# Angtian/VoGE

Hardware: AMD Instinct MI355X
Metric: forward+backward frames/sec at 512^2, 50k Gaussians; ray-trace HBM GB/s vs peak (higher is better)
Workload: dtype f32; 1 GPU; cfg3_50k_512: 50000 random Gaussians (scalar sigmas), 512x512, K=40, max_point_per_bin=-1, fwd+bwd (grads to verts, sigmas, colors); launch=hip graph replay, 4 consecutive steps per graph launch, parallelism=1 gpu

## Files before the change

### __graft_entry__.py

```python
import os
import subprocess
import sys

ROOT = os.path.dirname(os.path.abspath(__file__))
if ROOT not in sys.path:
    sys.path.insert(0, ROOT)


def build() -> None:
    subprocess.check_call(["make", "-C", os.path.join(ROOT, "voge_amd", "csrc"), "-B", "-j2", "all"])
    import oracle
    oracle.build(force=True)
    import voge_amd
    lib = voge_amd.load_library()
    assert lib.voge_abi_version() == 7
    from oracle import build_ref
    build_ref.build(force=True)


def smoke() -> None:
    import numpy as np
    import torch
    import oracle
    from oracle import camera_np
    from voge_amd.Meshes import GaussianMeshes
    from voge_amd.Renderer import GaussianRenderer, GaussianRenderSettings, to_white_background
    from voge_amd.cameras import PerspectiveCameras
    from voge_amd import scenes

    assert torch.cuda.is_available(), "smoke() needs a HIP device"
    dev = "cuda:0"
    verts, sig, cols = scenes.random_gaussians(600, seed=1, r_lo=0.08, r_hi=0.16)
    H = W = 64
    R, T = camera_np.look_at_view_transform(3.5, 15.0, 40.0)
    cams = PerspectiveCameras(focal_length=60.0, principal_point=((32.0, 32.0),), image_size=((H, W),), device=dev)
    st = GaussianRenderSettings(image_size=(H, W), max_assign=16, max_point_per_bin=-1)
    renderer = GaussianRenderer(cams, st).to(dev)
    gm = GaussianMeshes(torch.from_numpy(verts), torch.from_numpy(sig)).to(dev)
    colors = torch.from_numpy(cols).to(dev).requires_grad_(True)
    frag = renderer(gm, R=torch.from_numpy(R).to(dev), T=torch.from_numpy(T).to(dev))
    img = to_white_background(frag, colors)
    img.sum().backward()
    torch.cuda.synchronize()
    ref = oracle.render(verts, sig, cols, R, T, 60.0, (32.0, 32.0), (H, W), K=16)
    same = (frag.vert_index.cpu().numpy() == np.where(ref["idx"] < 0, 0, ref["idx"])).all(-1)
    err = np.abs(img.detach().cpu().numpy() - ref["image"])[same].max()
    assert same.mean() > 0.99 and err < 1e-4, (same.mean(), err)
    assert torch.isfinite(gm.verts.grad).all() and gm.verts.grad.abs().max() > 0
    print(f"smoke ok: {same.mean() * 100:.2f}% pixels identical index lists, max image err {err:.2e}")


if __name__ == "__main__":
    build()
    if len(sys.argv) > 1 and sys.argv[1] == "smoke":
        smoke()
```

### voge_amd/ops.py

```python
import math
import os
import struct

import torch

from . import _lib


_raw_stream = getattr(torch._C, "_cuda_getCurrentRawStream", None)
_get_dev = getattr(torch._C, "_cuda_getDevice", None) or torch.cuda.current_device
_set_dev = getattr(torch._C, "_cuda_setDevice", None) or torch.cuda.set_device


def _stream():
    if _raw_stream is not None:
        return _raw_stream(_get_dev())
    return torch.cuda.current_stream().cuda_stream


class _on:
    __slots__ = ("idx", "prev")

    def __init__(self, device):
        self.idx = device.index if device.index is not None else _get_dev()
        self.prev = -1

    def __enter__(self):
        cur = _get_dev()
        if cur != self.idx:
            self.prev = cur
            _set_dev(self.idx)

    def __exit__(self, *exc):
        if self.prev >= 0:
            _set_dev(self.prev)
        return False


def _dev(t, dtype, name):
    if not isinstance(t, torch.Tensor):
        raise TypeError(f"{name} must be a torch.Tensor")
    if not t.is_cuda:
        raise _lib.VogeHipError(
            f"{name} is on {t.device}: the VoGE hot path runs on a HIP device only (no CPU fallback)")
    if t.dtype != dtype:
        t = t.to(dtype)
    return t.contiguous()


def _p(t):
    return None if t is None else t.data_ptr()


_WS = {}


def _workspace(dev, nbytes):
    nbytes = max(int(nbytes), 16)
    if torch.cuda.is_current_stream_capturing():
        return torch.empty((nbytes,), dtype=torch.uint8, device=dev)
    key = (dev.index if dev.index is not None else _get_dev(), _stream())
    ws = _WS.get(key)
    if ws is None or ws.numel() < nbytes:
        ws = _WS[key] = torch.empty((nbytes,), dtype=torch.uint8, device=dev)
    return ws


def release_workspaces(device=None):
    idx = None if device is None else (torch.device(device).index if torch.device(device).index is not None else _get_dev())
    for key in [k for k in _WS if idx is None or k[0] == idx]:
        del _WS[key]


class _GeneralPreamble(torch.autograd.Function):

    @staticmethod
    def forward(ctx, verts, sigmas, origin):
        lib = _lib.load()
        v_c, s_c, o_c = _dev(verts, torch.float32, "verts"), _dev(sigmas, torch.float32, "sigmas"), _dev(origin, torch.float32, "origin")
        B = o_c.shape[0]
        shared_v = v_c.dim() == 2
        N = v_c.shape[-2]
        kind = 2 if tuple(s_c.shape[-2:]) == (3, 3) and s_c.dim() >= 3 else 1
        shared_s = s_c.dim() == (3 if kind == 2 else 2)
        assert v_c.shape[-1] == 3 and (shared_v or v_c.shape[0] == B) and o_c.shape == (B, 3)
        assert s_c.shape[-1] == 3 and s_c.shape[-(kind + 1)] == N and (shared_s or s_c.shape[0] == B)
        mus = torch.empty((B * N, 3), dtype=torch.float32, device=v_c.device)
        isg = torch.empty((B * N, 3, 3), dtype=torch.float32, device=v_c.device)
        with _on(v_c.device):
            rc = lib.voge_general_preamble_fwd(_p(v_c), _p(s_c), _p(o_c), B, N, int(shared_v), int(shared_s), kind, _p(mus), _p(isg),
                                               _stream())
        _lib.check(rc, "voge_general_preamble_fwd")
        ctx.meta = (B, N, shared_v, shared_s, kind, tuple(v_c.shape), tuple(s_c.shape))
        ctx.set_materialize_grads(False)
        return mus, isg

    @staticmethod
    def backward(ctx, g_mus, g_isg):
        lib = _lib.load()
        B, N, shared_v, shared_s, kind, vshape, sshape = ctx.meta
        if ctx.needs_input_grad[2]:
            raise _lib.VogeHipError("the fused preamble carries no gradient for the camera centre")
        g_v = g_s = None
        gm = None if g_mus is None else _dev(g_mus, torch.float32, "grad_mus")
        ga = None if g_isg is None else _dev(g_isg, torch.float32, "grad_isigmas")
        dev = (gm if gm is not None else ga)
        if dev is None:
            return None, None, None
        dev = dev.device
        if ctx.needs_input_grad[0] and gm is not None:
            g_v = torch.empty(vshape, dtype=torch.float32, device=dev)
        if ctx.needs_input_grad[1] and ga is not None:
            g_s = torch.empty(sshape, dtype=torch.float32, device=dev)
        if g_v is not None or g_s is not None:
            with _on(dev):
                rc = lib.voge_general_preamble_bwd(_p(gm if g_v is not None else None), _p(ga if g_s is not None else None), B, N,
                                                   int(shared_v), int(shared_s), kind, _p(g_v), _p(g_s), _stream())
            _lib.check(rc, "voge_general_preamble_bwd")
        return g_v, g_s, None


def general_preamble(verts, sigmas, origin):
    return _GeneralPreamble.apply(verts, sigmas, origin)


def trace_pool_usage(dev, B, N, H, W):
    import ctypes
    lib = _lib.load()
    dev = torch.device(dev)
    with _on(dev):
        nbytes = lib.voge_trace_workspace_bytes(B, N, H, W)
        ws = _workspace(dev, nbytes)
        used, cap = ctypes.c_int(0), ctypes.c_int(0)
        torch.cuda.current_stream(dev).synchronize()
        _lib.check(lib.voge_trace_pool_usage(_p(ws), nbytes, B, N, H, W, ctypes.byref(used), ctypes.byref(cap)), "voge_trace_pool_usage")
    return used.value, cap.value


def _tag_index(sel_idx, cnt, n_index):
    if cnt is not None:
        sel_idx.voge_hit_count = (cnt, sel_idx._version)
    sel_idx.voge_index_bound = (int(n_index), sel_idx._version)


def carry_tags(src, dst):
    if dst is src or not (isinstance(dst, torch.Tensor) and dst.is_cuda and dst.is_contiguous()
                          and dst.data_ptr() == src.data_ptr() and dst.numel() == src.numel() and dst.dtype == src.dtype):
        return dst
    tag = getattr(src, "voge_hit_count", None)
    if tag is not None:
        dst.voge_hit_count = (tag[0].view(dst.shape[:-1]), tag[1])
    for name in ("voge_index_bound", "voge_through"):
        tag = getattr(src, name, None)
        if tag is not None:
# ... 315 lines not shown
        lib = _lib.load()
        act, dsd = torch.empty_like(ln), torch.empty_like(ln)
        K = idx.shape[-1]
        with _on(ln.device):
            rc = lib.voge_fragment_act_dsd_iso(_p(records), _p(rays), _p(idx), _p(ln), _p(cnt), idx.numel() // K, K, P,
                                               _p(act), _p(dsd), _stream())
        _lib.check(rc, "voge_fragment_act_dsd_iso")
        cell[0], cell[1] = act, dsd
    return cell[0], cell[1]


def fragments(mode, p0, p1, origin, rays, cam_fwd, thr_act, n_assign, sigma_mode=0, occ=1.0):
    weight, sel_idx, valid, sel_len, cnt, records, sel_act, sel_dsd = _Fragments.apply(
        mode, p0, p1, origin, rays, cam_fwd, thr_act, n_assign, sigma_mode, occ)
    if (p0.requires_grad or p1.requires_grad) and torch.is_grad_enabled():
        B = rays.shape[0]
        N = p0.shape[-2] if mode == 2 else p0.shape[0] // max(B, 1)
        rays_d, len_d = rays.detach(), sel_len.detach()
        weight.voge_through = dict(
            mode=int(mode), sigma_mode=int(sigma_mode), shared=bool(mode == 2 and p0.dim() == 2), occ=float(occ), B=B, N=N,
            records=records, rays=rays_d, act=sel_act, dsd=sel_dsd, len=len_d, cnt=cnt, idx=sel_idx,
            sigmas=p1.detach(), means=p0.detach(), p0=p0, p1=p1, rays_requires_grad=bool(rays.requires_grad),
            versions=(weight._version, len_d._version, rays_d._version, sel_idx._version))
    return weight, sel_idx, valid, sel_len


LAZY_COMPOSITE = os.environ.get("VOGE_LAZY_COMPOSITE", "1") != "0"


class _TraceLean(torch.autograd.Function):

    @staticmethod
    def forward(ctx, mode, p0, p1, origin, rays, cam_fwd, thr_act, n_assign, sigma_mode):
        p0_c, p1_c, o_c, rays_c, fwd, B, N, H, W, shared = _trace_inputs(mode, p0, p1, origin, rays, cam_fwd)
        K, dev = int(n_assign), rays_c.device
        sel_idx = torch.empty((B, H, W, K), dtype=torch.int32, device=dev)
        sel_len = torch.empty((B, H, W, K), dtype=torch.float32, device=dev)
        cnt = torch.empty((B, H, W), dtype=torch.int32, device=dev)
        records = torch.empty((B * N, 12 if mode == 0 else 4), dtype=torch.float32, device=dev)
        _sweep(mode, p0_c, p1_c, o_c, shared, sigma_mode, rays_c, fwd, B, N, H, W, K, thr_act, 1.0, sel_idx, sel_len, None, None, cnt,
               None, None, records)
        ctx.save_for_backward(p0_c, p1_c, rays_c, sel_len)
        ctx.sel_idx, ctx.cnt, ctx.records = sel_idx, cnt, records
        ctx.meta = (int(mode), int(sigma_mode), bool(shared), B, N)
        _tag_index(sel_idx, cnt, B * N)
        ctx.mark_non_differentiable(sel_idx, cnt, records)
        ctx.set_materialize_grads(False)
        return sel_idx, sel_len, cnt, records

    @staticmethod
    def backward(ctx, _g_idx, g_len, _g_cnt, _g_rec):
        if g_len is None:
            return (None,) * 9
        p0, p1, rays, ln = ctx.saved_tensors
        mode, sigma_mode, shared, B, N = ctx.meta
        if ctx.needs_input_grad[4] or ctx.needs_input_grad[3]:
            raise _lib.VogeHipError("deferred-composite fragments carry no gradient for the rays / the camera centre; "
                                    "VOGE_LAZY_COMPOSITE=0 (or rays that require grad at render time) selects the eager chain")
        g0, g1 = _fragment_bwd(mode, p0, p1, ctx.records, shared, sigma_mode, rays, ctx.sel_idx, ctx.cnt, B, N, (p0, p1), ln, None, ln,
                               None, None, g_len, 1.0)
        return None, g0, g1, None, None, None, None, None, None


def _plain(t_, dtype, name):
    if not t_.is_cuda:
        raise _lib.VogeHipError(f"{name} is on {t_.device}: the VoGE hot path runs on a HIP device only (no CPU fallback)")
    if t_.dtype != dtype or not t_.is_contiguous():
        t_ = t_.detach().to(dtype).contiguous()
    return t_


def _sigma_kind(sigmas):
    kind = 2 if tuple(sigmas.shape[-2:]) == (3, 3) and sigmas.dim() >= 3 else 1
    return kind, sigmas.dim() == (3 if kind == 2 else 2)


def _plain16(t_, name):
    t_ = _plain(t_, torch.float32, name)
    return t_ if t_.data_ptr() % 16 == 0 else t_.detach().clone()


def _frame_trace(verts, sigmas, R, T, focal, pp, band, W, behind, thr_act, n_assign, sigma_mode, occ, origin_out, gen, quats=None):
    lib = _lib.load()
    v_c, s_c = _plain(verts, torch.float32, "verts"), _plain(sigmas, torch.float32, "sigmas")
    R_c, T_c = _plain(R, torch.float32, "R"), _plain(T, torch.float32, "T")
    f_c, p_c = _plain(focal, torch.float32, "focal_length"), _plain(pp, torch.float32, "principal_point")
    B = R_c.shape[0]
    row0, h, stripe_h, pitch = band
    shared = v_c.dim() == 2
    N, K, dev = v_c.shape[-2], int(n_assign), v_c.device
    assert R_c.shape == (B, 3, 3) and T_c.shape == (B, 3) and f_c.shape == (B, 2) and p_c.shape == (B, 2)
    assert v_c.shape[-1] == 3 and (shared or v_c.shape[0] == B)
    if quats is not None:
        q_c = _plain16(quats, "quats")
        shared_s = s_c.dim() == 2
        assert tuple(s_c.shape[-2:]) == (N, 3) and q_c.shape == s_c.shape[:-1] + (4,) and (shared_s or s_c.shape[0] == B)
        assert sigma_mode in (1, 2)
        nrec, form = 12, (0, int(sigma_mode), False, (3, int(shared), int(shared_s)))
    elif gen:
        kind, shared_s = _sigma_kind(s_c)
        assert s_c.shape[-(kind + 1)] == N and s_c.shape[-1] == 3 and (shared_s or s_c.shape[0] == B)
        nrec, form = (8 if kind == 1 else 12), (0, 0, False, (kind, int(shared), int(shared_s)))
    else:
        assert s_c.shape == v_c.shape[:-1]
        nrec, form = 4, (2, int(sigma_mode), shared, None)
    empty = torch.empty
    sel_idx = empty((B, h, W, K), dtype=torch.int32, device=dev)
    sel_len = empty((B, h, W, K), dtype=torch.float32, device=dev)
    cnt = empty((B, h, W), dtype=torch.int32, device=dev)
    records = empty((B * N, nrec), dtype=torch.float32, device=dev)
    rays = empty((B, h, W, 3), dtype=torch.float32, device=dev)
    with _on(dev):
        nbytes = lib.voge_trace_workspace_bytes(B, N, h, W)
        ws = _workspace(dev, nbytes)
        cam = (R_c.data_ptr(), T_c.data_ptr(), f_c.data_ptr(), p_c.data_ptr(), int(row0), int(stripe_h), int(pitch), int(bool(behind)), B,
               N, int(h), int(W), K, float(thr_act), ws.data_ptr(), nbytes, sel_idx.data_ptr(), sel_len.data_ptr(), cnt.data_ptr(),
               records.data_ptr(), rays.data_ptr(), _p(origin_out), _stream())
        if quats is not None:
            rc = lib.voge_frame_trace_fwd_ori(v_c.data_ptr(), s_c.data_ptr(), q_c.data_ptr(), int(shared), int(shared_s), int(sigma_mode), *cam)
        elif gen:
            rc = lib.voge_frame_trace_fwd_gen(v_c.data_ptr(), s_c.data_ptr(), int(shared), int(shared_s), kind, *cam)
        else:
            rc = lib.voge_frame_trace_fwd_iso(v_c.data_ptr(), s_c.data_ptr(), int(shared), int(sigma_mode), *cam)
    if rc:
        _lib.check(rc, "voge_frame_trace_fwd")
    _tag_index(sel_idx, cnt, B * N)
    lz = LazyComposite.__new__(LazyComposite)
    lz.mode, lz.sigma_mode, lz.shared, lz.gen = form
    (lz.occ, lz.B, lz.N, lz.K, lz.p0, lz.p1, lz.sel_idx, lz.sel_len, lz.cnt, lz.records, lz.rays, lz.rays_version, lz.grad_mode,
     lz.idx_version, lz.p0_version, lz.frame) = (float(occ), B, N, K, verts, sigmas, sel_idx, sel_len, cnt, records, rays, 0,
                                                 torch.is_grad_enabled(), sel_idx._version, verts._version, True)
    lz.p2 = quats
    lz.p12_version = None if quats is None else (sigmas._version, quats._version)
    return sel_idx, sel_len, lz


def frame_trace(verts, sigmas, R, T, focal, pp, band, W, behind, thr_act, n_assign, sigma_mode, occ, origin_out=None):
    return _frame_trace(verts, sigmas, R, T, focal, pp, band, W, behind, thr_act, n_assign, sigma_mode, occ, origin_out, False)


def frame_trace_gen(verts, sigmas, R, T, focal, pp, band, W, behind, thr_act, n_assign, occ, origin_out=None):
    return _frame_trace(verts, sigmas, R, T, focal, pp, band, W, behind, thr_act, n_assign, 0, occ, origin_out, True)


def frame_trace_ori(verts, scales, quats, R, T, focal, pp, band, W, behind, thr_act, n_assign, sigma_mode, occ, origin_out=None):
    return _frame_trace(verts, scales, R, T, focal, pp, band, W, behind, thr_act, n_assign, sigma_mode, occ, origin_out, True, quats)


def _frame_gen_bwd(lz, form, attr, weight, ad, ln, rgb, wsum, bg, thr, g, gs0, gs1, g_hitlen, acc=None):
    lz.check()
    lib = _lib.load()
    kind, shared_v, shared_s = lz.gen
    dev = ln.device
    B, H, W = lz.cnt.shape
    K, P = lz.K, lz.B * lz.N
    g0 = torch.empty(lz.p0.shape, dtype=torch.float32, device=dev)
    g1 = torch.empty(lz.p1.shape, dtype=torch.float32, device=dev)
    g_attr = None if attr is None else torch.empty_like(attr)
    g2 = None
    C, Nattr = (0, 0) if attr is None else (attr.shape[1], attr.shape[0])
    with _on(dev):
        zeroed = acc is not None
        if acc is None:
            nbytes = lib.voge_frame_bwd_gen_acc_bytes(P)
            acc = _workspace(dev, nbytes)
        else:
            nbytes = acc.numel()
        tail = (_p(lz.rays), _p(attr), _p(lz.sel_idx), _p(lz.cnt), _p(weight), _p(ad[0]), _p(ln), _p(ad[1]), _p(rgb), _p(wsum), _p(bg),
                float(thr), _p(g), gs0, gs1, _p(g_hitlen), lz.occ, lz.B, lz.N, B * H, W, K, C, Nattr, _p(acc), nbytes, int(zeroed), _p(g0),
                _p(g1))
        if kind == 3:
            g2 = torch.empty(lz.p2.shape, dtype=torch.float32, device=dev)
            rc = lib.voge_frame_bwd_ori(form, _p(lz.records), _p(_plain(lz.p1, torch.float32, "scales")), _p(_plain16(lz.p2, "quats")),
                                        shared_v, shared_s, lz.sigma_mode, *tail, _p(g2), _p(g_attr), _stream())
        else:
            rc = lib.voge_frame_bwd_gen(form, _p(lz.records), shared_v, shared_s, kind, *tail, _p(g_attr), _stream())
    _lib.check(rc, "voge_frame_bwd_ori" if kind == 3 else "voge_frame_bwd_gen")
    return g0, g1, g2, g_attr


class _HitLength(torch.autograd.Function):

    @staticmethod
    def forward(ctx, p0, p1, sel_len, lz, p2=None):
        ctx.lz = lz
        ctx.save_for_backward(p1)
        ctx.set_materialize_grads(False)
        return sel_len.view_as(sel_len)

    @staticmethod
    def backward(ctx, g_len):
        if g_len is None:
            return None, None, None, None, None
        lz = ctx.lz
        (p1,) = ctx.saved_tensors
        if lz.gen is None:
            p1 = _dev(p1, torch.float32, "sigmas")
        g0, g1, g2 = _lazy_fragment_bwd(lz, p1, lz.sel_len, lz.sel_len, None, g_len=g_len, occ=1.0)
        return g0, g1, None, None, g2


FRAME_PATH = os.environ.get("VOGE_FRAME_PATH", "1") != "0"
FRAME_DIRECT_BWD = os.environ.get("VOGE_FRAME_DIRECT_BWD", "1") != "0"


def frame_eligible(verts, sigmas, R, T, focal, pp, n_assign, numel):
    if not (LAZY_COMPOSITE and FRAME_PATH) or n_assign > _lib.MAX_K or os.environ.get("VOGE_FRAGMENTS_KEEP_ACT_DSD", "0") == "1":
        return False
# ... 106 lines not shown
            per = 32 if lz.gen is None else (48 if lz.gen[0] == 1 else 64)
        return torch.empty((lz.B * lz.N * per,), dtype=torch.uint8, device=lz.sel_idx.device)
    return None


def _composite_fwd(lz, sel_len, need, attr=None, bg=None, thr=-1.0, rgb=None, img=None, wsum=None, sil=None, acc=None):
    lib = _lib.load()
    idx, K = lz.sel_idx, lz.K
    npix = idx.numel() // K
    C, Nattr = (0, 0) if attr is None else (attr.shape[1], attr.shape[0])
    nacc = 0 if acc is None else acc.numel()
    weight = torch.empty_like(sel_len)
    valid = torch.empty(idx.shape[:-1], dtype=torch.int64, device=idx.device)
    with _on(idx.device):
        ad = _general_act_dsd(lz, sel_len, need)
        src = (_p(idx), _p(lz.cnt), _p(sel_len), _p(lz.records), _p(lz.rays), lz.occ)
        args = src + (_p(attr), _p(bg), float(thr), npix, K, C, Nattr, _p(weight), _p(valid), _p(rgb), _p(img), _p(wsum))
        if lz.gen is not None:
            rc = lib.voge_frame_shade_fwd_rec(1 if lz.gen[0] == 1 else 2, *args, _p(sil), _p(ad[0]), _p(ad[1]), _p(acc), nacc, _stream())
        elif attr is None and lz.mode == 0:
            rc = lib.voge_composite_fwd_rec(*src, npix, K, _p(weight), _p(valid), _p(ad[0]), _p(ad[1]), _stream())
        elif attr is None:
            rc = lib.voge_composite_fwd_iso(*src, npix, K, _p(weight), _p(valid), _stream())
        elif lz.mode == 0:
            rc = lib.voge_composite_shade_fwd_rec(*args, _p(ad[0]), _p(ad[1]), _stream())
        elif sil is not None or acc is not None:
            rc = lib.voge_frame_shade_fwd_iso(*args, _p(sil), _p(acc), nacc, _stream())
        else:
            rc = lib.voge_composite_shade_fwd_iso(*args, _stream())
    _lib.check(rc, "voge_composite_fwd (from the records)")
    weight.voge_act_dsd = ad
    return weight, valid, ad


class _CompositeLean(torch.autograd.Function):

    @staticmethod
    def forward(ctx, p0, p1, sel_len, lz, p2=None):
        weight, valid, ctx.ad = _composite_fwd(lz, sel_len, any(ctx.needs_input_grad))
        ctx.save_for_backward(_dev(p1, torch.float32, "sigmas"), sel_len, weight)
        ctx.lz = lz
        ctx.mark_non_differentiable(valid)
        ctx.set_materialize_grads(False)
        return weight, valid

    @staticmethod
    def backward(ctx, g_weight, _g_valid):
        if g_weight is None:
            return None, None, None, None, None
        p1, ln, weight = ctx.saved_tensors
        g0, g1, g2 = _lazy_fragment_bwd(ctx.lz, p1, weight, ln, g_weight, ctx.ad)
        return g0, g1, None, None, g2


def _shade_bwd(mode, means, sigmas, records, shared, sigma_mode, rays, cnt, occ, B, N, like, attr, idx, weight, act, ln, dsd, rgb,
               wsum, bg, thr, go, gs_pix, gs_c, acc=None):
    lib = _lib.load()
    _, H, W, K = idx.shape
    Nattr, C = attr.shape
    dev = idx.device
    g_attr = torch.empty_like(attr)
    g0 = torch.empty(like[0].shape, dtype=torch.float32, device=dev)
    g1 = torch.empty(like[1].shape, dtype=torch.float32, device=dev)
    image = (_p(rgb), _p(wsum), _p(bg), thr, _p(go), gs_pix, gs_c, occ)
    sizes = (B * H, W, K, C, Nattr)
    grads = (_p(g0), _p(g1), _p(g_attr))
    with _on(dev):
        if acc is not None:
            rc = lib.voge_frame_shade_bwd_iso(_p(records), _p(sigmas), int(shared), sigma_mode, _p(rays), _p(attr), _p(idx), _p(cnt),
                                              _p(weight), _p(ln), *image, B, N, *sizes, _p(acc), acc.numel(), *grads, _stream())
        else:
            nbytes = lib.voge_fragment_bwd_workspace_bytes(B * N)
            ws = _workspace(dev, nbytes)
            slots = (_p(attr), _p(idx), _p(cnt), _p(weight), _p(act), _p(ln), _p(dsd), *image)
            if mode == 0:
                rc = lib.voge_fragment_shade_bwd(_p(means), _p(sigmas), _p(rays), *slots, B * N, *sizes, _p(ws), nbytes, *grads, _stream())
            else:
                rc = lib.voge_fragment_shade_bwd_iso(_p(records), _p(sigmas), int(shared), sigma_mode, _p(rays), *slots, B, N, *sizes,
                                                     _p(ws), nbytes, *grads, _stream())
    _lib.check(rc, "voge_fragment_shade_bwd")
    return g0, g1, g_attr


class _CompositeShade(torch.autograd.Function):

    @staticmethod
    def forward(ctx, attr, p0, p1, sel_len, lz, bg, thr, p2=None):
        attr_c = _dev(attr, torch.float32, "colors")
        bg_c = _dev(bg, torch.float32, "background_color")
        idx = lz.sel_idx
        Nattr, C = attr_c.shape
        assert bg_c.numel() == C
        check_index_range(idx, Nattr)
        rgb = torch.empty(idx.shape[:-1] + (C,), dtype=torch.float32, device=idx.device)
        img = torch.empty_like(rgb)
        wsum = torch.empty(idx.shape[:-1], dtype=torch.float32, device=idx.device)
        ctx.gbuf = _frame_acc(lz, any(ctx.needs_input_grad[:3]) or ctx.needs_input_grad[-1])
        weight, valid, ctx.ad = _composite_fwd(lz, sel_len, any(ctx.needs_input_grad), attr_c, bg_c, thr, rgb, img, wsum, acc=ctx.gbuf)
        ctx.save_for_backward(attr_c, _dev(p1, torch.float32, "sigmas"), sel_len, weight, rgb, bg_c, wsum)
        ctx.lz, ctx.thr = lz, float(thr)
        ctx.mark_non_differentiable(valid)
        ctx.set_materialize_grads(False)
        return img, weight, valid

    @staticmethod
    def backward(ctx, g_img, g_weight, _g_valid):
        attr, p1, ln, weight, rgb, bg, wsum = ctx.saved_tensors
        lz = ctx.lz
        lz.check()
        g_attr = g0 = g1 = g2 = None
        if g_img is not None:
            go, gs_pix, gs_c = _grad_layout(g_img, attr.shape[1])
            gbuf, ctx.gbuf = ctx.gbuf, None
            if lz.gen is not None:
                g0, g1, g2, g_attr = _frame_gen_bwd(lz, 0, attr, weight, ctx.ad, ln, rgb, wsum, bg, ctx.thr, go, gs_pix, gs_c, None, acc=gbuf)
            else:
                g0, g1, g_attr = _shade_bwd(lz.mode, lz.means() if lz.mode == 0 else None, p1, lz.records, lz.shared, lz.sigma_mode,
                                            lz.rays, lz.cnt, lz.occ, lz.B, lz.N, (lz.p0, lz.p1), attr, lz.sel_idx, weight, ctx.ad[0], ln,
                                            ctx.ad[1], rgb, wsum, bg, ctx.thr, go, gs_pix, gs_c, gbuf)
        if g_weight is not None:
            h0, h1, h2 = _lazy_fragment_bwd(lz, p1, weight, ln, g_weight, ctx.ad)
            g0, g1, g2 = (h0, h1, h2) if g0 is None else (g0 + h0, g1 + h1, None if h2 is None else g2 + h2)
        need = ctx.needs_input_grad
        return ((g_attr if need[0] else None), (g0 if need[1] else None), (g1 if need[2] else None), None, None, None, None,
                (g2 if need[7] else None))


def _merge_bwd(lz, p1, attr, weight, ad, ln, go, gs_pix, gs_c, gws, wsum_fwd, acc):
    lib = _lib.load()
    idx = lz.sel_idx
    B, H, W, K = idx.shape
    Nattr, C = attr.shape
    dev = idx.device
    g_attr = torch.empty_like(attr)
    g0 = torch.empty(lz.p0.shape, dtype=torch.float32, device=dev)
    g1 = torch.empty(lz.p1.shape, dtype=torch.float32, device=dev)
    grad = (_p(go), gs_pix, gs_c, _p(gws))
    sizes = (B * H, W, K, C, Nattr)
    grads = (_p(g0), _p(g1), _p(g_attr))
    with _on(dev):
        if acc is not None:
            rc = lib.voge_frame_merge_bwd_iso(_p(lz.records), _p(p1), int(lz.shared), lz.sigma_mode, _p(lz.rays), _p(attr), _p(idx),
                                              _p(lz.cnt), _p(weight), _p(ln), *grad, _p(wsum_fwd), lz.occ, lz.B, lz.N, *sizes, _p(acc),
                                              acc.numel(), *grads, _stream())
        else:
            nbytes = lib.voge_fragment_bwd_workspace_bytes(lz.B * lz.N)
            ws = _workspace(dev, nbytes)
            slots = (_p(attr), _p(idx), _p(lz.cnt), _p(weight), _p(ad[0]), _p(ln), _p(ad[1]), *grad, lz.occ)
            if lz.mode == 0:
                rc = lib.voge_fragment_merge_bwd(_p(lz.means()), _p(p1), _p(lz.rays), *slots, lz.B * lz.N, *sizes, _p(ws), nbytes, *grads,
                                                 _stream())
            else:
                rc = lib.voge_fragment_merge_bwd_iso(_p(lz.records), _p(p1), int(lz.shared), lz.sigma_mode, _p(lz.rays), *slots, lz.B,
                                                     lz.N, *sizes, _p(ws), nbytes, *grads, _stream())
    _lib.check(rc, "voge_fragment_merge_bwd")
    return g0, g1, g_attr


class _CompositeMerge(torch.autograd.Function):

    @staticmethod
    def forward(ctx, attr, p0, p1, sel_len, lz, p2=None):
        attr_c = _dev(attr, torch.float32, "vert_attr")
        idx = lz.sel_idx
        Nattr, C = attr_c.shape
        check_index_range(idx, Nattr)
        rgb = torch.empty(idx.shape[:-1] + (C,), dtype=torch.float32, device=idx.device)
        wsum = torch.empty(idx.shape[:-1], dtype=torch.float32, device=idx.device)
        sil = torch.empty_like(wsum) if lz.frame else None
        ctx.gbuf = _frame_acc(lz, any(ctx.needs_input_grad[:3]) or ctx.needs_input_grad[-1])
        weight, valid, ctx.ad = _composite_fwd(lz, sel_len, any(ctx.needs_input_grad), attr_c, None, -1.0, rgb, None, wsum, sil, ctx.gbuf)
        ctx.save_for_backward(attr_c, _dev(p1, torch.float32, "sigmas"), sel_len, weight, wsum)
        ctx.lz = lz
        ctx.mark_non_differentiable(valid)
        ctx.set_materialize_grads(False)
        return rgb, wsum, weight, valid, sil

    @staticmethod
    def backward(ctx, g_rgb, g_wsum, g_weight, _g_valid, g_sil=None):
        attr, p1, ln, weight, wsum = ctx.saved_tensors
        lz = ctx.lz
        lz.check()
        idx = lz.sel_idx
        C = attr.shape[1]
        g_attr = g0 = g1 = g2 = None
        wsum_fwd = None
        if g_sil is not None:
            if g_wsum is None and (ctx.gbuf is not None or lz.gen is not None):
                g_wsum, wsum_fwd = g_sil, wsum
            else:
                passed = g_sil * torch.where(wsum < 1, 1.0, torch.where(wsum == 1, 0.5, 0.0))
                g_wsum = passed if g_wsum is None else g_wsum + passed
        if g_rgb is not None or g_wsum is not None:
            if g_rgb is None:
                g_rgb = torch.zeros(idx.shape[:-1] + (C,), dtype=torch.float32, device=idx.device)
            go, gs_pix, gs_c = _grad_layout(g_rgb, C)
# ... 1155 lines not shown
```

Baseline: 4635 frames/s.

## Move eager frame trace and shade host glue into a compiled C++ extension

Adds a pybind11/ATen extension that validates tensors, allocates outputs and workspace, and calls the libvoge_hip trace, shade forward and shade backward entries directly, bypassing the Python/ctypes wrappers. ops.py routes the isotropic frame path through it when it is available. This is meant to cut per-call Python and ctypes dispatch cost on the eager path. It adds a build dependency tied to the torch version and a parallel code path that must stay consistent with the Python one.

```diff
diff --git a/__graft_entry__.py b/__graft_entry__.py
--- a/__graft_entry__.py
+++ b/__graft_entry__.py
@@ -8,12 +8,14 @@
 
 
 def build() -> None:
-    subprocess.check_call(["make", "-C", os.path.join(ROOT, "voge_amd", "csrc"), "-B", "-j2", "all"])
+    subprocess.check_call(["make", "-C", os.path.join(ROOT, "voge_amd", "csrc"), "-B", "-j3", "all", "PYTHON=" + sys.executable])
     import oracle
     oracle.build(force=True)
     import voge_amd
     lib = voge_amd.load_library()
     assert lib.voge_abi_version() == 7
+    from voge_amd import _host
+    _host.load()
     from oracle import build_ref
     build_ref.build(force=True)
 
diff --git a/voge_amd/_host.py b/voge_amd/_host.py
--- /dev/null
+++ b/voge_amd/_host.py
@@ -0,0 +1,61 @@
+import ctypes
+import importlib
+import os
+import warnings
+
+import torch
+
+from . import _lib
+
+INTERFACE = 1
+ENTRIES = ("voge_trace_workspace_bytes", "voge_error_string", "voge_frame_trace_fwd_iso", "voge_frame_shade_fwd_iso",
+           "voge_frame_shade_bwd_iso")
+
+
+class HostExtUnavailable(_lib.VogeHipError):
+    """voge_amd._host_ext is not built, was built against another torch, or speaks another interface."""
+
+
+def load(torch_version=None):
+    want = torch.__version__ if torch_version is None else torch_version
+    try:
+        mod = importlib.import_module("voge_amd._host_ext")
+    except ImportError as e:
+        raise HostExtUnavailable(f"voge_amd._host_ext cannot be imported ({e}); `make -C voge_amd/csrc host` builds it") from e
+    if getattr(mod, "TORCH_VERSION", None) != want:
+        raise HostExtUnavailable(f"voge_amd._host_ext was built against torch {getattr(mod, 'TORCH_VERSION', '?')}, this is "
+                                 f"torch {want}; `make -C voge_amd/csrc -B host` rebuilds it")
+    if getattr(mod, "INTERFACE", None) != INTERFACE:
+        raise HostExtUnavailable(f"voge_amd._host_ext speaks interface {getattr(mod, 'INTERFACE', '?')}, the package {INTERFACE}")
+    return mod
+
+
+def resolve(setting):
+    if setting == "0":
+        return None
+    try:
+        return load()
+    except HostExtUnavailable as e:
+        if setting == "1":
+            raise
+        warnings.warn(f"{e} -- the eager frame takes the Python host route (VOGE_HOST_EXT=0 says so without this warning)",
+                      RuntimeWarning, stacklevel=2)
+        return None
+
+
+_bound = None
+_entries = {}
+
+
+def bound(mod, lib, names):
+    global _bound, _entries
+    if lib is not _bound:
+        entries = {name: getattr(lib, name) for name in ENTRIES}
+        if not all(isinstance(fn, ctypes._CFuncPtr) for fn in entries.values()):
+            return None
+        mod.bind(*(ctypes.cast(entries[name], ctypes.c_void_p).value for name in ENTRIES), _lib.VogeHipError)
+        _bound, _entries = lib, entries
+    for name in names:
+        if getattr(lib, name) is not _entries[name]:
+            return None
+    return mod
diff --git a/voge_amd/csrc/host/frame_args.h b/voge_amd/csrc/host/frame_args.h
--- /dev/null
+++ b/voge_amd/csrc/host/frame_args.h
@@ -0,0 +1,171 @@
+#pragma once
+#include <cstddef>
+#include <cstdint>
+
+namespace voge_host {
+
+constexpr int kInterface = 1;
+
+typedef void *stream_t;
+
+constexpr int kErrUnbound = -100;
+constexpr int kErrSize = -101;
+constexpr int kErrNull = -102;
+constexpr int kErrAlign = -103;
+
+inline const char *error_string(int code) {
+  switch (code) {
+    case kErrUnbound: return "the host extension is not bound to a loaded libvoge_hip";
+    case kErrSize: return "a size is out of range";
+    case kErrNull: return "a required pointer is null";
+    case kErrAlign: return "the backward's accumulator must be 16-byte aligned and a multiple of 16 bytes";
+    default: return "unknown host-extension error";
+  }
+}
+
+typedef size_t (*trace_workspace_bytes_fn)(int B, int N, int H, int W);
+typedef const char *(*error_string_fn)(int code);
+typedef int (*frame_trace_fwd_iso_fn)(const float *verts, const float *sigmas, int shared, int sigma_mode, const float *R,
+                                      const float *T, const float *focal, const float *pp, int row0, int stripe_h, int pitch,
+                                      int behind, int B, int N, int h, int W, int K, float thr_act, void *workspace,
+                                      size_t workspace_bytes, int32_t *idx, float *len, int32_t *cnt, float *records, float *rays,
+                                      float *origin, stream_t stream);
+typedef int (*frame_shade_fwd_iso_fn)(int32_t *idx, const int32_t *cnt, const float *len, const float *records, const float *rays,
+                                      float occ, const float *colors, const float *bg, float thr, long npix, int K, int C,
+                                      long Nattr, float *weight, int64_t *valid_num, float *rgb, float *img, float *wsum,
+                                      float *sil, void *bwd_acc, size_t bwd_acc_bytes, stream_t stream);
+typedef int (*frame_shade_bwd_iso_fn)(const float *records, const float *sigmas, int shared, int sigma_mode, const float *rays,
+                                      const float *colors, const int32_t *idx, const int32_t *cnt, const float *weight,
+                                      const float *len, const float *rgb, const float *wsum, const float *bg, float thr,
+                                      const float *g_img, long g_stride_pix, long g_stride_c, float occ, int B, int N, long nrows,
+                                      int W, int K, int C, long Nattr, void *acc_zeroed, size_t acc_bytes, float *g_verts,
+                                      float *g_sigmas, float *g_colors, stream_t stream);
+
+struct EntryTable {
+  trace_workspace_bytes_fn trace_workspace_bytes = nullptr;
+  error_string_fn error_string = nullptr;
+  frame_trace_fwd_iso_fn frame_trace_fwd_iso = nullptr;
+  frame_shade_fwd_iso_fn frame_shade_fwd_iso = nullptr;
+  frame_shade_bwd_iso_fn frame_shade_bwd_iso = nullptr;
+};
+
+constexpr int kMaxShadeK = 128;
+constexpr int kAccBytesPerGaussian = 32;
+
+struct TraceArgs {
+  const float *verts = nullptr, *sigmas = nullptr;
+  int shared = 0, sigma_mode = 0;
+  const float *R = nullptr, *T = nullptr, *focal = nullptr, *pp = nullptr;
+  int row0 = 0, stripe_h = 0, pitch = 0, behind = 0;
+  int B = 0, N = 0, h = 0, W = 0, K = 0;
+  float thr_act = 0.f;
+  void *workspace = nullptr;
+  size_t workspace_bytes = 0;
+  int32_t *idx = nullptr;
+  float *len = nullptr;
+  int32_t *cnt = nullptr;
+  float *records = nullptr;
+  float *rays = nullptr;
+  float *origin = nullptr;
+  stream_t stream = nullptr;
+};
+
+struct TraceSizes {
+  long slots = 0, pixels = 0, records = 0, rays = 0;
+};
+
+inline int trace_sizes(int B, int N, int h, int W, int K, TraceSizes *out) {
+  if (B <= 0 || N <= 0 || h <= 0 || W <= 0 || K <= 0) return kErrSize;
+  out->pixels = static_cast<long>(B) * h * W;
+  out->slots = out->pixels * K;
+  out->records = static_cast<long>(B) * N * 4;
+  out->rays = out->pixels * 3;
+  return 0;
+}
+
+inline int trace_workspace_bytes(const EntryTable &t, int B, int N, int h, int W, size_t *out) {
+  if (!t.trace_workspace_bytes) return kErrUnbound;
+  if (B <= 0 || N <= 0 || h <= 0 || W <= 0) return kErrSize;
+  size_t n = t.trace_workspace_bytes(B, N, h, W);
+  *out = n < 16 ? size_t(16) : n;
+  return 0;
+}
+
+inline int frame_trace_iso(const EntryTable &t, const TraceArgs &a) {
+  if (!t.frame_trace_fwd_iso) return kErrUnbound;
+  TraceSizes sz;
+  if (int rc = trace_sizes(a.B, a.N, a.h, a.W, a.K, &sz)) return rc;
+  if (a.row0 < 0 || a.stripe_h < 0 || a.pitch < 0) return kErrSize;
+  if (!a.verts || !a.sigmas || !a.R || !a.T || !a.focal || !a.pp) return kErrNull;
+  if (!a.workspace || !a.idx || !a.len || !a.cnt || !a.records || !a.rays) return kErrNull;
+  return t.frame_trace_fwd_iso(a.verts, a.sigmas, a.shared ? 1 : 0, a.sigma_mode, a.R, a.T, a.focal, a.pp, a.row0, a.stripe_h,
+                               a.pitch, a.behind ? 1 : 0, a.B, a.N, a.h, a.W, a.K, a.thr_act, a.workspace, a.workspace_bytes,
+                               a.idx, a.len, a.cnt, a.records, a.rays, a.origin, a.stream);
+}
+
+struct ShadeFwdArgs {
+  int32_t *idx = nullptr;
+  const int32_t *cnt = nullptr;
+  const float *len = nullptr, *records = nullptr, *rays = nullptr;
+  float occ = 1.f;
+  const float *colors = nullptr, *bg = nullptr;
+  float thr = -1.f;
+  long npix = 0;
+  int K = 0, C = 0;
+  long Nattr = 0;
+  float *weight = nullptr;
+  int64_t *valid_num = nullptr;
+  float *rgb = nullptr, *img = nullptr;
+  float *wsum = nullptr;
+  void *acc = nullptr;
+  size_t acc_bytes = 0;
+  stream_t stream = nullptr;
+};
+
+inline int frame_shade_fwd_iso(const EntryTable &t, const ShadeFwdArgs &a) {
+  if (!t.frame_shade_fwd_iso) return kErrUnbound;
+  if (a.npix <= 0 || a.K <= 0 || a.K > kMaxShadeK || (a.C != 3 && a.C != 4) || a.Nattr <= 0) return kErrSize;
+  if (!a.idx || !a.cnt || !a.len || !a.records || !a.rays || !a.colors || !a.bg) return kErrNull;
+  if (!a.weight || !a.valid_num || !a.rgb || !a.img || !a.wsum) return kErrNull;
+  size_t nacc = a.acc ? a.acc_bytes : 0;
+  if (nacc && ((nacc & 15) || (reinterpret_cast<uintptr_t>(a.acc) & 15))) return kErrAlign;
+  return t.frame_shade_fwd_iso(a.idx, a.cnt, a.len, a.records, a.rays, a.occ, a.colors, a.bg, a.thr, a.npix, a.K, a.C, a.Nattr,
+                               a.weight, a.valid_num, a.rgb, a.img, a.wsum, nullptr, a.acc, nacc, a.stream);
+}
+
+struct ShadeBwdArgs {
+  const float *records = nullptr, *sigmas = nullptr;
+  int shared = 0, sigma_mode = 0;
+  const float *rays = nullptr, *colors = nullptr;
+  const int32_t *idx = nullptr, *cnt = nullptr;
+  const float *weight = nullptr, *len = nullptr, *rgb = nullptr, *wsum = nullptr, *bg = nullptr;
+  float thr = -1.f;
+  const float *g_img = nullptr;
+  long g_stride_pix = 0, g_stride_c = 0;
+  float occ = 1.f;
+  int B = 0, N = 0;
+  long nrows = 0;
+  int W = 0, K = 0, C = 0;
+  long Nattr = 0;
+  void *acc = nullptr;
+  size_t acc_bytes = 0;
+  float *g_verts = nullptr, *g_sigmas = nullptr, *g_colors = nullptr;
+  stream_t stream = nullptr;
+};
+
+inline int frame_shade_bwd_iso(const EntryTable &t, const ShadeBwdArgs &a) {
+  if (!t.frame_shade_bwd_iso) return kErrUnbound;
+  if (a.B <= 0 || a.N <= 0 || a.nrows <= 0 || a.W <= 0 || a.K <= 0 || a.K > kMaxShadeK || (a.C != 3 && a.C != 4) || a.Nattr <= 0)
+    return kErrSize;
+  if (a.g_stride_pix < 0 || a.g_stride_c < 0) return kErrSize;
+  if (!a.records || !a.sigmas || !a.rays || !a.colors || !a.idx || !a.cnt || !a.weight || !a.len || !a.rgb || !a.wsum || !a.bg)
+    return kErrNull;
+  if (!a.g_img || !a.acc || !a.g_verts || !a.g_sigmas || !a.g_colors) return kErrNull;
+  if ((a.acc_bytes & 15) || (reinterpret_cast<uintptr_t>(a.acc) & 15)) return kErrAlign;
+  if (a.acc_bytes < static_cast<size_t>(a.B) * a.N * kAccBytesPerGaussian) return kErrSize;
+  return t.frame_shade_bwd_iso(a.records, a.sigmas, a.shared ? 1 : 0, a.sigma_mode, a.rays, a.colors, a.idx, a.cnt, a.weight,
+                               a.len, a.rgb, a.wsum, a.bg, a.thr, a.g_img, a.g_stride_pix, a.g_stride_c, a.occ, a.B, a.N,
+                               a.nrows, a.W, a.K, a.C, a.Nattr, a.acc, a.acc_bytes, a.g_verts, a.g_sigmas, a.g_colors, a.stream);
+}
+
+}
diff --git a/voge_amd/csrc/host/host_ext.cpp b/voge_amd/csrc/host/host_ext.cpp
--- /dev/null
+++ b/voge_amd/csrc/host/host_ext.cpp
@@ -0,0 +1,302 @@
+#include <ATen/ATen.h>
+#include <c10/hip/HIPFunctions.h>
+#include <c10/hip/HIPGraphsC10Utils.h>
+#include <c10/hip/HIPGuard.h>
+#include <c10/hip/HIPStream.h>
+#include <torch/csrc/utils/pybind.h>
+
+#include <map>
+#include <optional>
+#include <string>
+#include <utility>
+
+#include "frame_args.h"
+
+namespace py = pybind11;
+using voge_host::EntryTable;
+
+#ifndef VOGE_TORCH_VERSION
+#error "VOGE_TORCH_VERSION: the Makefile bakes in torch.__version__ of the build"
+#endif
+#define VOGE_STR_(x) #x
+#define VOGE_STR(x) VOGE_STR_(x)
+
+namespace {
+
+EntryTable g_table;
+PyObject *g_error_type = nullptr;
+
+[[noreturn]] void raise(PyObject *type, const std::string &msg) {
+  PyErr_SetString(type ? type : PyExc_RuntimeError, msg.c_str());
+  throw py::error_already_set();
+}
+
+[[noreturn]] void raise_voge(const std::string &msg) { raise(g_error_type, msg); }
+
+void expect(bool ok, const char *what) {
+  if (!ok) raise(PyExc_AssertionError, what);
+}
+
+void check(int rc, const char *what) {
+  if (rc == 0) return;
+  if (rc <= voge_host::kErrUnbound) raise_voge(std::string(what) + ": " + voge_host::error_string(rc));
+  const char *msg = g_table.error_string ? g_table.error_string(rc) : "?";
+  raise_voge(std::string(what) + " failed with code " + std::to_string(rc) + ": " + (msg ? msg : "?"));
+}
+
+void need_hip(const at::Tensor &t, const char *name) {
+  if (!t.is_cuda())
+    raise_voge(std::string(name) + " is on " + t.device().str() + ": the VoGE hot path runs on a HIP device only (no CPU fallback)");
+}
+
+at::Tensor plain(const at::Tensor &t, const char *name) {
+  need_hip(t, name);
+  if (t.scalar_type() != at::kFloat || !t.is_contiguous()) return t.detach().to(at::kFloat).contiguous();
+  return t;
+}
+
+at::Tensor dev(const at::Tensor &t, const char *name) {
+  need_hip(t, name);
+  return (t.scalar_type() != at::kFloat ? t.to(at::kFloat) : t).contiguous();
+}
+
+struct OnDevice {
+  c10::DeviceIndex prev = -1;
+  explicit OnDevice(c10::DeviceIndex idx) {
+    c10::DeviceIndex cur = c10::hip::current_device();
+    if (cur != idx) {
+      prev = cur;
+      c10::hip::set_device(idx);
+    }
+  }
+  ~OnDevice() {
+    if (prev >= 0) c10::hip::set_device(prev);
+  }
+};
+
+void *raw_stream(c10::DeviceIndex idx) { return static_cast<void *>(c10::hip::getCurrentHIPStream(idx).stream()); }
+
+typedef std::map<std::pair<int, uintptr_t>, at::Tensor> WorkspaceMap;
+WorkspaceMap &workspaces() {
+  static WorkspaceMap *m = new WorkspaceMap();
+  return *m;
+}
+uintptr_t g_last_workspace = 0;
+
+at::Tensor workspace(const c10::Device &device, void *stream, size_t nbytes) {
+  auto opts = at::TensorOptions().dtype(at::kByte).device(device);
+  at::Tensor ws;
+  if (c10::hip::currentStreamCaptureStatusMayInitCtx() != c10::hip::CaptureStatus::None) {
+    ws = at::empty({static_cast<int64_t>(nbytes)}, opts);
+  } else {
+    auto key = std::make_pair(static_cast<int>(device.index()), reinterpret_cast<uintptr_t>(stream));
+    auto &m = workspaces();
+    auto it = m.find(key);
+    if (it == m.end() || static_cast<size_t>(it->second.numel()) < nbytes) {
+      if (it != m.end()) m.erase(it);
+      it = m.emplace(key, at::empty({static_cast<int64_t>(nbytes)}, opts)).first;
+    }
+    ws = it->second;
+  }
+  g_last_workspace = reinterpret_cast<uintptr_t>(ws.data_ptr());
+  return ws;
+}
+
+at::Tensor workspace_for(int device, size_t nbytes) {
+  if (nbytes < 16) nbytes = 16;
+  auto idx = static_cast<c10::DeviceIndex>(device);
+  return workspace(c10::Device(c10::DeviceType::CUDA, idx), raw_stream(idx), nbytes);
+}
+
+void release_workspaces(int device) {
+  auto &m = workspaces();
+  for (auto it = m.begin(); it != m.end();) it = (device < 0 || it->first.first == device) ? m.erase(it) : std::next(it);
+}
+
+uintptr_t cached_workspace(int device, uintptr_t stream) {
+  auto &m = workspaces();
+  auto it = m.find(std::make_pair(device, stream));
+  return it == m.end() ? 0 : reinterpret_cast<uintptr_t>(it->second.data_ptr());
+}
+
+py::list cached_workspaces() {
+  py::list out;
+  for (auto &kv : workspaces())
+    out.append(py::make_tuple(kv.first.first, kv.first.second, reinterpret_cast<uintptr_t>(kv.second.data_ptr()), kv.second.numel()));
+  return out;
+}
+
+template <typename F>
+F entry(uintptr_t addr) {
+  return reinterpret_cast<F>(addr);
+}
+
+void bind(uintptr_t trace_workspace_bytes, uintptr_t error_string, uintptr_t frame_trace_fwd_iso, uintptr_t frame_shade_fwd_iso,
+          uintptr_t frame_shade_bwd_iso, py::object error_type) {
+  g_table.trace_workspace_bytes = entry<voge_host::trace_workspace_bytes_fn>(trace_workspace_bytes);
+  g_table.error_string = entry<voge_host::error_string_fn>(error_string);
+  g_table.frame_trace_fwd_iso = entry<voge_host::frame_trace_fwd_iso_fn>(frame_trace_fwd_iso);
+  g_table.frame_shade_fwd_iso = entry<voge_host::frame_shade_fwd_iso_fn>(frame_shade_fwd_iso);
+  g_table.frame_shade_bwd_iso = entry<voge_host::frame_shade_bwd_iso_fn>(frame_shade_bwd_iso);
+  PyObject *prev = g_error_type;
+  g_error_type = error_type.inc_ref().ptr();
+  Py_XDECREF(prev);
+}
+
+inline const float *fp(const at::Tensor &t) { return static_cast<const float *>(t.data_ptr()); }
+inline float *fpm(const at::Tensor &t) { return static_cast<float *>(t.data_ptr()); }
+inline int32_t *ip(const at::Tensor &t) { return static_cast<int32_t *>(t.data_ptr()); }
+
+py::tuple frame_trace_iso(const at::Tensor &verts, const at::Tensor &sigmas, const at::Tensor &R, const at::Tensor &T,
+                          const at::Tensor &focal, const at::Tensor &pp, int row0, int h, int stripe_h, int pitch, int W, bool behind,
+                          double thr_act, int K, int sigma_mode, const std::optional<at::Tensor> &origin_out) {
+  at::Tensor v = plain(verts, "verts"), s = plain(sigmas, "sigmas");
+  at::Tensor Rc = plain(R, "R"), Tc = plain(T, "T");
+  at::Tensor fc = plain(focal, "focal_length"), pc = plain(pp, "principal_point");
+  expect(Rc.dim() >= 1, "R must be [B,3,3]");
+  const int64_t B = Rc.size(0);
+  expect(v.dim() >= 2, "verts must be [N,3] or [B,N,3]");
+  const bool shared = v.dim() == 2;
+  const int64_t N = v.size(-2);
+  expect(Rc.sizes() == at::IntArrayRef({B, 3, 3}) && Tc.sizes() == at::IntArrayRef({B, 3}) && fc.sizes() == at::IntArrayRef({B, 2}) &&
+             pc.sizes() == at::IntArrayRef({B, 2}),
+         "R [B,3,3], T [B,3], focal_length [B,2] and principal_point [B,2] must agree");
+  expect(v.size(-1) == 3 && (shared || v.size(0) == B), "verts must be [N,3] or [B,N,3]");
+  expect(s.sizes() == v.sizes().slice(0, v.dim() - 1), "scalar sigmas must be shaped like verts without its last axis");
+  expect(B <= INT32_MAX && N <= INT32_MAX, "B and N must fit 32 bits");
+
+  const c10::Device device = v.device();
+  auto f32 = at::TensorOptions().dtype(at::kFloat).device(device);
+  auto i32 = at::TensorOptions().dtype(at::kInt).device(device);
+  at::Tensor sel_idx = at::empty({B, h, W, K}, i32);
+  at::Tensor sel_len = at::empty({B, h, W, K}, f32);
+  at::Tensor cnt = at::empty({B, h, W}, i32);
+  at::Tensor records = at::empty({B * N, 4}, f32);
+  at::Tensor rays = at::empty({B, h, W, 3}, f32);
+
+  voge_host::TraceArgs a;
+  int rc;
+  {
+    OnDevice on(device.index());
+    size_t nbytes = 0;
+    check(voge_host::trace_workspace_bytes(g_table, static_cast<int>(B), static_cast<int>(N), h, W, &nbytes), "voge_frame_trace_fwd");
+    a.stream = raw_stream(device.index());
+    at::Tensor ws = workspace(device, a.stream, nbytes);
+    a.verts = fp(v), a.sigmas = fp(s), a.shared = shared, a.sigma_mode = sigma_mode;
+    a.R = fp(Rc), a.T = fp(Tc), a.focal = fp(fc), a.pp = fp(pc);
+    a.row0 = row0, a.stripe_h = stripe_h, a.pitch = pitch, a.behind = behind;
+    a.B = static_cast<int>(B), a.N = static_cast<int>(N), a.h = h, a.W = W, a.K = K;
+    a.thr_act = static_cast<float>(thr_act);
+    a.workspace = ws.data_ptr(), a.workspace_bytes = nbytes;
+    a.idx = ip(sel_idx), a.len = fpm(sel_len), a.cnt = ip(cnt), a.records = fpm(records), a.rays = fpm(rays);
+    a.origin = origin_out.has_value() && origin_out->defined() ? fpm(*origin_out) : nullptr;
+    rc = voge_host::frame_trace_iso(g_table, a);
+  }
+  check(rc, "voge_frame_trace_fwd");
+  return py::make_tuple(sel_idx, sel_len, cnt, records, rays, B, N, shared);
+}
+
+py::tuple frame_shade_fwd_iso(const at::Tensor &attr, const at::Tensor &bg, double thr, const at::Tensor &sel_idx, const at::Tensor &cnt,
+                              const at::Tensor &sel_len, const at::Tensor &records, const at::Tensor &rays, double occ, int64_t P,
+                              bool need_acc) {
+  at::Tensor attr_c = dev(attr, "colors");
+  at::Tensor bg_c = dev(bg, "background_color");
+  expect(attr_c.dim() == 2 && sel_idx.dim() >= 2, "colors must be [N,C], the index list [..,K]");
+  const int64_t Nattr = attr_c.size(0), C = attr_c.size(1);
+  expect(bg_c.numel() == C, "the background colour must have one value per channel");
+  const int64_t K = sel_idx.size(-1);
+  expect(K > 0, "K must be positive");
+  const int64_t npix = sel_idx.numel() / K;
+
+  const c10::Device device = sel_idx.device();
+  auto f32 = at::TensorOptions().dtype(at::kFloat).device(device);
+  std::vector<int64_t> pix(sel_idx.sizes().begin(), sel_idx.sizes().end() - 1);
+  std::vector<int64_t> pix_c(pix);
+  pix_c.push_back(C);
+  at::Tensor rgb = at::empty(pix_c, f32);
+  at::Tensor img = at::empty(pix_c, f32);
+  at::Tensor wsum = at::empty(pix, f32);
+  at::Tensor weight = at::empty_like(sel_len);
+  at::Tensor valid = at::empty(pix, at::TensorOptions().dtype(at::kLong).device(device));
+  at::Tensor acc;
+  if (need_acc) acc = at::empty({P * voge_host::kAccBytesPerGaussian}, at::TensorOptions().dtype(at::kByte).device(device));
+
+  voge_host::ShadeFwdArgs a;
+  a.idx = ip(sel_idx), a.cnt = ip(cnt), a.len = fp(sel_len), a.records = fp(records), a.rays = fp(rays);
+  a.occ = static_cast<float>(occ), a.colors = fp(attr_c), a.bg = fp(bg_c), a.thr = static_cast<float>(thr);
+  a.npix = npix, a.K = static_cast<int>(K), a.C = static_cast<int>(C), a.Nattr = Nattr;
+  a.weight = fpm(weight), a.valid_num = static_cast<int64_t *>(valid.data_ptr());
+  a.rgb = fpm(rgb), a.img = fpm(img), a.wsum = fpm(wsum);
+  if (acc.defined()) a.acc = acc.data_ptr(), a.acc_bytes = static_cast<size_t>(acc.numel());
+  int rc;
+  {
+    OnDevice on(device.index());
+    a.stream = raw_stream(device.index());
+    rc = voge_host::frame_shade_fwd_iso(g_table, a);
+  }
+  check(rc, "voge_composite_fwd (from the records)");
+  return py::make_tuple(attr_c, bg_c, rgb, img, wsum, weight, valid, acc.defined() ? py::cast(acc) : py::none());
+}
+
+py::tuple frame_shade_bwd_iso(const at::Tensor &records, const at::Tensor &sigmas, bool shared, int sigma_mode, const at::Tensor &rays,
+                              const at::Tensor &attr, const at::Tensor &idx, const at::Tensor &cnt, const at::Tensor &weight,
+                              const at::Tensor &ln, const at::Tensor &rgb, const at::Tensor &wsum, const at::Tensor &bg, double thr,
+                              const at::Tensor &g_img, double occ, int B, int N, const at::Tensor &p0, const at::Tensor &p1,
+                              const at::Tensor &acc) {
+  expect(idx.dim() == 4 && attr.dim() == 2, "the index list must be [B,h,W,K], the colors [N,C]");
+  const int64_t H = idx.size(1), W = idx.size(2), K = idx.size(3);
+  const int64_t Nattr = attr.size(0), C = attr.size(1);
+
+  at::Tensor go = g_img;
+  long gs_pix = C, gs_c = 1;
+  bool broadcast = g_img.scalar_type() == at::kFloat && g_img.is_cuda();
+  for (int64_t st : g_img.strides()) broadcast = broadcast && st == 0;
+  if (broadcast) {
+    gs_pix = gs_c = 0;
+  } else {
+    go = dev(g_img, "grad_image");
+  }
+
+  const c10::Device device = idx.device();
+  auto f32 = at::TensorOptions().dtype(at::kFloat).device(device);
+  at::Tensor g_attr = at::empty_like(attr);
+  at::Tensor g0 = at::empty(p0.sizes(), f32);
+  at::Tensor g1 = at::empty(p1.sizes(), f32);
+
+  voge_host::ShadeBwdArgs a;
+  a.records = fp(records), a.sigmas = fp(sigmas), a.shared = shared, a.sigma_mode = sigma_mode;
+  a.rays = fp(rays), a.colors = fp(attr), a.idx = ip(idx), a.cnt = ip(cnt);
+  a.weight = fp(weight), a.len = fp(ln), a.rgb = fp(rgb), a.wsum = fp(wsum), a.bg = fp(bg);
+  a.thr = static_cast<float>(thr), a.g_img = fp(go), a.g_stride_pix = gs_pix, a.g_stride_c = gs_c, a.occ = static_cast<float>(occ);
+  a.B = B, a.N = N, a.nrows = static_cast<long>(B) * H, a.W = static_cast<int>(W), a.K = static_cast<int>(K);
+  a.C = static_cast<int>(C), a.Nattr = Nattr;
+  a.acc = acc.data_ptr(), a.acc_bytes = static_cast<size_t>(acc.numel());
+  a.g_verts = fpm(g0), a.g_sigmas = fpm(g1), a.g_colors = fpm(g_attr);
+  int rc;
+  {
+    OnDevice on(device.index());
+    a.stream = raw_stream(device.index());
+    rc = voge_host::frame_shade_bwd_iso(g_table, a);
+  }
+  check(rc, "voge_fragment_shade_bwd");
+  return py::make_tuple(g0, g1, g_attr);
+}
+
+}
+
+PYBIND11_MODULE(_host_ext, m) {
+  m.doc() = "Host glue of the eager frame path, compiled (see voge_amd/csrc/host/host_ext.cpp)";
+  m.attr("TORCH_VERSION") = VOGE_STR(VOGE_TORCH_VERSION);
+  m.attr("INTERFACE") = voge_host::kInterface;
+  m.def("bind", &bind, "Bind the table of entry addresses of the loaded libvoge_hip and the error type");
+  m.def("frame_trace_iso", &frame_trace_iso);
+  m.def("frame_shade_fwd_iso", &frame_shade_fwd_iso);
+  m.def("frame_shade_bwd_iso", &frame_shade_bwd_iso);
+  m.def("workspace", &workspace_for, "The scratch of (device, its current stream), at least nbytes: ops._workspace's rules");
+  m.def("release_workspaces", &release_workspaces, "Drop the cached scratch buffers (device < 0: all)");
+  m.def("cached_workspace", &cached_workspace, "data_ptr of the scratch cached for (device, raw stream), or 0");
+  m.def("cached_workspaces", &cached_workspaces, "[(device, raw stream, data_ptr, bytes)] of every cached scratch buffer");
+  m.def("last_workspace", []() { return g_last_workspace; }, "data_ptr of the scratch the last trace used");
+  m.def("current_stream", [](int device) { return reinterpret_cast<uintptr_t>(raw_stream(static_cast<c10::DeviceIndex>(device))); },
+        "Raw handle of the current stream of a device, as the three calls read it");
+}
diff --git a/voge_amd/ops.py b/voge_amd/ops.py
--- a/voge_amd/ops.py
+++ b/voge_amd/ops.py
@@ -4,7 +4,7 @@
 
 import torch
 
-from . import _lib
+from . import _host, _lib
 
 
 _raw_stream = getattr(torch._C, "_cuda_getCurrentRawStream", None)
@@ -35,6 +35,23 @@
         if self.prev >= 0:
             _set_dev(self.prev)
         return False
+
+
+_host_ext = _host.resolve(os.environ.get("VOGE_HOST_EXT"))
+HOST_EXT = _host_ext is not None
+
+
+_EXT_TRACE = ("voge_frame_trace_fwd_iso", "voge_trace_workspace_bytes")
+_EXT_SHADE_FWD = ("voge_frame_shade_fwd_iso",)
+_EXT_SHADE_BWD = ("voge_frame_shade_bwd_iso",)
+
+
+def _ext(lib, entries):
+    if not HOST_EXT:
+        return None
+    if _host_ext is None:
+        raise _lib.VogeHipError("ops.HOST_EXT is on but voge_amd._host_ext was not loaded (VOGE_HOST_EXT=0 at import?)")
+    return _host.bound(_host_ext, lib, entries)
 
 
 def _dev(t, dtype, name):
@@ -57,6 +74,8 @@
 
 def _workspace(dev, nbytes):
     nbytes = max(int(nbytes), 16)
+    if _host_ext is not None:
+        return _host_ext.workspace(dev.index if dev.index is not None else _get_dev(), nbytes)
     if torch.cuda.is_current_stream_capturing():
         return torch.empty((nbytes,), dtype=torch.uint8, device=dev)
     key = (dev.index if dev.index is not None else _get_dev(), _stream())
@@ -70,6 +89,8 @@
     idx = None if device is None else (torch.device(device).index if torch.device(device).index is not None else _get_dev())
     for key in [k for k in _WS if idx is None or k[0] == idx]:
         del _WS[key]
+    if _host_ext is not None:
+        _host_ext.release_workspaces(-1 if idx is None else idx)
 
 
 class _GeneralPreamble(torch.autograd.Function):
@@ -551,6 +572,14 @@
 
 def _frame_trace(verts, sigmas, R, T, focal, pp, band, W, behind, thr_act, n_assign, sigma_mode, occ, origin_out, gen, quats=None):
     lib = _lib.load()
+    ext = _ext(lib, _EXT_TRACE) if not gen and quats is None else None
+    if ext is not None:
+        row0, h, stripe_h, pitch = band
+        K = int(n_assign)
+        sel_idx, sel_len, cnt, records, rays, B, N, shared = ext.frame_trace_iso(
+            verts, sigmas, R, T, focal, pp, int(row0), int(h), int(stripe_h), int(pitch), int(W), bool(behind), float(thr_act), K,
+            int(sigma_mode), origin_out)
+        return _frame_fragments(verts, sigmas, None, (2, int(sigma_mode), shared, None), occ, B, N, K, sel_idx, sel_len, cnt, records, rays)
     v_c, s_c = _plain(verts, torch.float32, "verts"), _plain(sigmas, torch.float32, "sigmas")
     R_c, T_c = _plain(R, torch.float32, "R"), _plain(T, torch.float32, "T")
     f_c, p_c = _plain(focal, torch.float32, "focal_length"), _plain(pp, torch.float32, "principal_point")
@@ -593,6 +622,10 @@
             rc = lib.voge_frame_trace_fwd_iso(v_c.data_ptr(), s_c.data_ptr(), int(shared), int(sigma_mode), *cam)
     if rc:
         _lib.check(rc, "voge_frame_trace_fwd")
+    return _frame_fragments(verts, sigmas, quats, form, occ, B, N, K, sel_idx, sel_len, cnt, records, rays)
+
+
+def _frame_fragments(verts, sigmas, quats, form, occ, B, N, K, sel_idx, sel_len, cnt, records, rays):
     _tag_index(sel_idx, cnt, B * N)
     lz = LazyComposite.__new__(LazyComposite)
     lz.mode, lz.sigma_mode, lz.shared, lz.gen = form
@@ -865,10 +898,28 @@
     return g0, g1, g_attr
 
 
+def _host_shade_route(lz, attr):
+    return (HOST_EXT and lz.frame and lz.gen is None and lz.mode == 2 and lz.K <= 128 and FRAME_DIRECT_BWD and attr.dim() == 2
+            and attr.shape[1] in (3, 4))
+
+
 class _CompositeShade(torch.autograd.Function):
 
     @staticmethod
     def forward(ctx, attr, p0, p1, sel_len, lz, bg, thr, p2=None):
+        ext = _ext(_lib.load(), _EXT_SHADE_FWD) if _host_shade_route(lz, attr) else None
+        if ext is not None:
+            check_index_range(lz.sel_idx, attr.shape[0])
+            need = ctx.needs_input_grad
+            attr_c, bg_c, rgb, img, wsum, weight, valid, ctx.gbuf = ext.frame_shade_fwd_iso(
+                attr, bg, float(thr), lz.sel_idx, lz.cnt, sel_len, lz.records, lz.rays, lz.occ, lz.B * lz.N,
+                bool(any(need[:3]) or need[-1]))
+            weight.voge_act_dsd = ctx.ad = (None, None)
+            ctx.save_for_backward(attr_c, _dev(p1, torch.float32, "sigmas"), sel_len, weight, rgb, bg_c, wsum)
+            ctx.lz, ctx.thr = lz, float(thr)
+            ctx.mark_non_differentiable(valid)
+            ctx.set_materialize_grads(False)
+            return img, weight, valid
         attr_c = _dev(attr, torch.float32, "colors")
         bg_c = _dev(bg, torch.float32, "background_color")
         idx = lz.sel_idx
@@ -893,8 +944,15 @@
         lz.check()
         g_attr = g0 = g1 = g2 = None
         if g_img is not None:
+            gbuf, ctx.gbuf = ctx.gbuf, None
+            ext = _ext(_lib.load(), _EXT_SHADE_BWD) if gbuf is not None and g_weight is None and _host_shade_route(lz, attr) else None
+            if ext is not None:
+                need = ctx.needs_input_grad
+                g0, g1, g_attr = ext.frame_shade_bwd_iso(lz.records, p1, lz.shared, lz.sigma_mode, lz.rays, attr, lz.sel_idx, lz.cnt,
+                                                         weight, ln, rgb, wsum, bg, ctx.thr, g_img, lz.occ, lz.B, lz.N, lz.p0, lz.p1, gbuf)
+                return ((g_attr if need[0] else None), (g0 if need[1] else None), (g1 if need[2] else None), None, None, None, None,
+                        None)
             go, gs_pix, gs_c = _grad_layout(g_img, attr.shape[1])
-            gbuf, ctx.gbuf = ctx.gbuf, None
             if lz.gen is not None:
                 g0, g1, g2, g_attr = _frame_gen_bwd(lz, 0, attr, weight, ctx.ad, ln, rgb, wsum, bg, ctx.thr, go, gs_pix, gs_c, None, acc=gbuf)
             else:
```

Result: no change. 4629 frames/s (-0.1%).
